# fakhirsh/path-tracer-python

Hardware: AMD Instinct MI355X
Metric: Msamples/s + achieved HBM GB/s, vol2_final_scene 800x800 at 1/2/4/8 MI355X (higher is better)
Workload: dtype f32; 1 GPU; vol2_final_scene 800x800 @ 16640 spp in total (260 steps x 64 spp), megakernel integrator, max_depth 50; scene=vol2_final_scene, width=800, height=800, variant=mk, traversal=stack, total_spp=16640, partition=tiles, rows_per_rank=800, max_depth=50, seed=0, parallelism=single GPU

## Files before the change

### path-tracer-python_amd/csrc/pt_abi.hip

```cpp
#include <hip/hip_runtime.h>

#include <cstdarg>
#include <cstdio>
#include <cstring>
#include <string>

#include "../../include/ptmi_wf_tiles.h"
#include "pt_args.hpp"
#include "pt_image.hpp"
#include "pt_launch.hpp"
#include "pt_prof.hpp"

namespace ptmi {

__global__ __launch_bounds__(kBlock) void clear_kernel(DevFrame fr, float* __restrict__ accum) {
  const int32_t npix = fr.w * fr.n_rows;
  for (int32_t i = (int32_t)(blockIdx.x * kBlock + threadIdx.x); i < npix; i += (int32_t)(gridDim.x * kBlock)) {
    int32_t lr = i / fr.w;
    int32_t px = fr.x0 + (i - lr * fr.w);
    int32_t py = frame_row(fr, lr);
    float* p = accum + 3 * ((size_t)py * (size_t)fr.width + (size_t)px);
    p[0] = 0.0f;
    p[1] = 0.0f;
    p[2] = 0.0f;
// ... 84 lines not shown
  if (s->shell != 0) {
    const int64_t off = ((int64_t)s->shell - 1) & ~(int64_t)1;
    if (s->shell < 0 || off % kNodeBytes != 0 || off / kNodeBytes >= s->n_inner)
      return fail(PTMI_EINVAL, "shell %d is not 1 + a node offset (multiple of %u, below %d nodes) + child index",
                  s->shell, kNodeBytes, s->n_inner);
  }
  std::memset(&d, 0, sizeof d);
  d.nodes = (const float4*)s->nodes;
  d.n_inner = s->n_inner;
  d.root_ref = (np > 0) ? s->root_ref : 0;
  for (int k = 0; k < 3; ++k) {
    d.root_min[k] = s->root_min[k];
    d.root_max[k] = s->root_max[k];
  }
  d.spheres = (const float4*)s->spheres;
  d.quads = (const float4*)s->quads;
  d.tris = (const float4*)s->tris;
  d.mats = (const float4*)s->mats;
  d.mat_base[kSphere] = 0;
  d.mat_base[kQuad] = s->num_spheres;
  d.mat_base[kTriangle] = s->num_spheres + s->num_quads;
  d.texels = s->texels;
  d.num_images = s->num_images;
  for (int k = 0; k < PTMI_MAX_IMAGES; ++k) {
    d.img_offset[k] = s->img_offset[k];
    d.img_w[k] = s->img_w[k];
    d.img_h[k] = s->img_h[k];
  }
  d.perlin_vec = (const float4*)s->perlin_vec;
  d.perlin_perm = s->perlin_perm;
  d.ref_nodes = (const float4*)s->ref_nodes;
  d.n_nodes = s->num_bvh_nodes;
  d.shell = s->max_leaf_depth <= 62 ? s->shell : 0;
  return PTMI_OK;
}

static int to_dev_frame(const ptmi_frame* f, DevFrame& d) {
  if (!f) return fail(PTMI_EINVAL, "frame is NULL");
  if (f->width <= 0 || f->height <= 0 || f->w <= 0 || f->h <= 0 || f->x0 < 0 || f->y0 < 0 ||
      f->x0 + f->w > f->width || f->y0 + f->h > f->height)
    return fail(PTMI_EINVAL, "bad window %d,%d %dx%d in %dx%d", f->x0, f->y0, f->w, f->h, f->width, f->height);
  if ((int64_t)f->width * (int64_t)f->height > (int64_t)0x7fffffff / 3)
    return fail(PTMI_ECAPACITY, "image too large");
  if (f->band_rows <= 0 || f->band_stride <= 0 || f->band_offset < 0 || f->band_offset >= f->band_stride)
    return fail(PTMI_EINVAL, "bad band partition");
  if (f->max_depth < 0 || f->max_depth > 255) return fail(PTMI_EINVAL, "max_depth must be in [0, 255]");
  std::memset(&d, 0, sizeof d);
  for (int k = 0; k < 3; ++k) {
    d.center[k] = f->cam.center[k];
    d.pixel00[k] = f->cam.pixel00[k];
    d.delta_u[k] = f->cam.delta_u[k];
    d.delta_v[k] = f->cam.delta_v[k];
    d.defocus_u[k] = f->cam.defocus_u[k];
    d.defocus_v[k] = f->cam.defocus_v[k];
    d.bg[k] = f->bg[k];
  }
  d.defocus_angle = f->cam.defocus_angle;
  d.max_depth = f->max_depth;
  d.seed = f->seed;
  d.width = f->width;
  d.height = f->height;
  d.x0 = f->x0;
  d.y0 = f->y0;
  d.w = f->w;
  d.h = f->h;
  d.band_rows = f->band_rows;
// ... 328 lines not shown
```

### path-tracer-python_amd/csrc/pt_device.hpp

```cpp
#pragma once
#include <hip/hip_runtime.h>
#include <stdint.h>

#include "../../include/ptmi.h"
#include "../../include/ptmi_math.h"
#include "../../include/ptmi_rng.h"

namespace ptmi {

constexpr float kTMin = 0.001f;
constexpr float kTMax = 1e10f;
constexpr int kRRMinDepth = 5;
constexpr float kRRMaxProb = 0.95f;
constexpr int kNumCounters = PTMI_NUM_COUNTERS;


struct FastDiv {
  uint64_t m;
  uint32_t sh, d;
};
static inline FastDiv fast_div(uint32_t d) {
  uint32_t l = 0;
  while ((1ull << l) < d) ++l;
  return FastDiv{((1ull << (32 + l)) / d) + 1ull, 32u + l, d};
}
__device__ __forceinline__ uint32_t fdiv(uint32_t n, const FastDiv& f) { return (uint32_t)(((uint64_t)n * f.m) >> f.sh); }
constexpr int kBlock = 256;

#ifndef PTMI_STRESS_WAVES
#define PTMI_STRESS_WAVES 0
#endif
constexpr int stress_waves(int w) { return PTMI_STRESS_WAVES > w ? PTMI_STRESS_WAVES : w; }

enum : int32_t { kSphere = 0, kTriangle = 1, kQuad = 2 };

struct DevScene {
  const float4* __restrict__ nodes;
  int32_t n_inner;
  int32_t root_ref;
  float root_min[3], root_max[3];
  const float4* __restrict__ spheres;
  const float4* __restrict__ quads;
  const float4* __restrict__ tris;
  const float4* __restrict__ mats;
  int32_t mat_base[3];
  const uint32_t* __restrict__ texels;
  int32_t num_images;
  int32_t img_offset[PTMI_MAX_IMAGES], img_w[PTMI_MAX_IMAGES], img_h[PTMI_MAX_IMAGES];
  const float4* __restrict__ perlin_vec;
  const int32_t* __restrict__ perlin_perm;
  const float4* __restrict__ ref_nodes;
  int32_t n_nodes;
  int32_t shell;
};

struct DevFrame {
  float center[3], pixel00[3], delta_u[3], delta_v[3], defocus_u[3], defocus_v[3];
  float defocus_angle;
  float bg[3];
  int32_t max_depth;
  uint32_t seed;
  int32_t width, height;
  int32_t x0, y0, w, h;
  int32_t band_rows, band_stride, band_offset;
  int32_t n_rows;
  int32_t traversal;
};

__device__ __forceinline__ int32_t leaf_type(int32_t ref) { return (ref >> 28) & 3; }
__device__ __forceinline__ int32_t leaf_index(int32_t ref) { return ref & 0x01ffffff; }
__device__ __forceinline__ int32_t leaf_class(int32_t ref) { return (ref >> 25) & 7; }

__device__ __forceinline__ int32_t frame_row(const DevFrame& fr, int32_t lr) {
  int32_t band = lr / fr.band_rows;
  int32_t within = lr - band * fr.band_rows;
  int32_t row = fr.y0 + (band * fr.band_stride + fr.band_offset) * fr.band_rows + within;
  return (row < fr.y0 + fr.h) ? row : -1;
}
// ... 86 lines not shown
  float z = sqrtf(1.0f - r2);
  float phi = PT_2PI_F * r1;
  float st = sqrtf(r2);
  float sp, cp;
  pt_sincosf(phi, &sp, &cp);
  float x = cp * st, y = sp * st;
  pt_v3 w = pt_normalize(n);
  pt_v3 a = (fabsf(w.x) < 0.9f) ? pt_v3f(1.0f, 0.0f, 0.0f)
            : (fabsf(w.y) < 0.9f) ? pt_v3f(0.0f, 1.0f, 0.0f) : pt_v3f(0.0f, 0.0f, 1.0f);
  pt_v3 v = pt_normalize(pt_cross(a, w));
  pt_v3 u = pt_cross(v, w);
  return pt_normalize(pt_add(pt_add(pt_scale(u, x), pt_scale(v, y)), pt_scale(w, z)));
}

__device__ __forceinline__ void get_ray(const DevFrame& fr, int32_t px, int32_t py, Rng& r, pt_v3& o,
                                        pt_v3& d) {
  float ox = r.next() - 0.5f;
  float oy = r.next() - 0.5f;
  pt_v3 p00 = pt_v3f(fr.pixel00[0], fr.pixel00[1], fr.pixel00[2]);
  pt_v3 du = pt_v3f(fr.delta_u[0], fr.delta_u[1], fr.delta_u[2]);
  pt_v3 dv = pt_v3f(fr.delta_v[0], fr.delta_v[1], fr.delta_v[2]);
  pt_v3 ps = pt_add(pt_add(p00, pt_scale(du, (float)px + ox)), pt_scale(dv, (float)py + oy));
  pt_v3 c = pt_v3f(fr.center[0], fr.center[1], fr.center[2]);
  o = c;
  if (fr.defocus_angle > 0.0f) {
    pt_v3 p = random_in_unit_disk(r);
    pt_v3 fu = pt_v3f(fr.defocus_u[0], fr.defocus_u[1], fr.defocus_u[2]);
    pt_v3 fv = pt_v3f(fr.defocus_v[0], fr.defocus_v[1], fr.defocus_v[2]);
    o = pt_add(pt_add(c, pt_scale(fu, p.x)), pt_scale(fv, p.y));
  }
  d = pt_sub(ps, o);
}

__device__ __forceinline__ bool pt_all4(bool a, bool b, bool c, bool d) {
  return __builtin_amdgcn_inverse_ballot_w64(__builtin_amdgcn_ballot_w64(a) & __builtin_amdgcn_ballot_w64(b) &
                                             __builtin_amdgcn_ballot_w64(c) & __builtin_amdgcn_ballot_w64(d));
}

__device__ __forceinline__ bool pt_all2(bool a, bool b) {
  return __builtin_amdgcn_inverse_ballot_w64(__builtin_amdgcn_ballot_w64(a) & __builtin_amdgcn_ballot_w64(b));
}


template <bool EXCL = false>
__device__ __forceinline__ bool hit_sphere_t(const float4 s, pt_v3 o, pt_v3 d, float tmin, float tmax,
                                             float& t) {
  pt_v3 c = pt_v3f(s.x, s.y, s.z);
  pt_v3 oc = pt_sub(c, o);
  float a = pt_dot(d, d);
  const float ra = pt_recip_for_div(a);
#define PT_SPH_DIV(x) pt_div_by((x), a, ra)
  float h = pt_dot(d, oc);
  float cc = pt_dot(oc, oc) - s.w * s.w;
  float disc = h * h - a * cc;
  if (disc >= 0.0f) {
    float sq = sqrtf(disc);
    float root = PT_SPH_DIV(h - sq);
    if (root < tmin || root > tmax) root = PT_SPH_DIV(h + sq);
    if (pt_all2(root >= tmin, EXCL ? root < tmax : root <= tmax)) { t = root; return true; }
  }
  return false;
#undef PT_SPH_DIV
}

template <bool EXCL = false>
__device__ __forceinline__ bool hit_quad_v(const float4 a, const float4 b, const float4 c, const float4 e, pt_v3 o,
                                           pt_v3 d, float tmin, float tmax, float& t) {
  pt_v3 n = pt_v3f(a.x, a.y, a.z);
  float denom = pt_dot(n, d);
  if (fabsf(denom) >= 1e-8f) {
    float tt = (a.w - pt_dot(n, o)) / denom;
    if (pt_all2(tt >= tmin, EXCL ? tt < tmax : tt <= tmax)) {
      pt_v3 Q = pt_v3f(b.x, b.y, b.z), u = pt_v3f(b.w, c.x, c.y), v = pt_v3f(c.z, c.w, e.x);
      pt_v3 w = pt_v3f(e.y, e.z, e.w);
      pt_v3 ip = pt_add(o, pt_scale(d, tt));
      pt_v3 pv = pt_sub(ip, Q);
      float alpha = pt_dot(w, pt_cross(pv, v));
      float beta = pt_dot(w, pt_cross(u, pv));
      if (pt_all4(alpha >= 0.0f, alpha <= 1.0f, beta >= 0.0f, beta <= 1.0f)) { t = tt; return true; }
    }
  }
  return false;
}

template <bool EXCL = false>
__device__ __forceinline__ bool hit_quad_t(const float4* __restrict__ q, pt_v3 o, pt_v3 d, float tmin,
                                           float tmax, float& t) {
  typedef float pt_f4 __attribute__((ext_vector_type(4)));
  pt_f4 A = ((const pt_f4*)q)[0], B = ((const pt_f4*)q)[1], C = ((const pt_f4*)q)[2], E = ((const pt_f4*)q)[3];
  asm volatile("" : "+v"(A), "+v"(B), "+v"(C), "+v"(E));
  return hit_quad_v<EXCL>(make_float4(A.x, A.y, A.z, A.w), make_float4(B.x, B.y, B.z, B.w),
                    make_float4(C.x, C.y, C.z, C.w), make_float4(E.x, E.y, E.z, E.w), o, d, tmin, tmax, t);
}

template <bool EXCL = false>
__device__ __forceinline__ bool hit_tri_v(const float4 a, const float4 b, const float4 c, pt_v3 o, pt_v3 d,
                                          float tmin, float tmax, float& t) {
  pt_v3 v0 = pt_v3f(a.x, a.y, a.z), e1 = pt_v3f(a.w, b.x, b.y), e2 = pt_v3f(b.z, b.w, c.x);
  pt_v3 hv = pt_cross(d, e2);
  float det = pt_dot(e1, hv);
  if (fabsf(det) >= 1e-8f) {
    float inv = 1.0f / det;
    pt_v3 s = pt_sub(o, v0);
    float u = inv * pt_dot(s, hv);
    if (pt_all2(u >= 0.0f, u <= 1.0f)) {
      pt_v3 q = pt_cross(s, e1);
      float v = inv * pt_dot(d, q);
      if (pt_all2(v >= 0.0f, u + v <= 1.0f)) {
        float tt = inv * pt_dot(e2, q);
        if (pt_all2(tt >= tmin, EXCL ? tt < tmax : tt <= tmax)) { t = tt; return true; }
      }
    }
  }
  return false;
}

template <bool EXCL = false>
__device__ __forceinline__ bool hit_tri_t(const float4* __restrict__ tr, pt_v3 o, pt_v3 d, float tmin,
                                          float tmax, float& t) {
  typedef float pt_f4 __attribute__((ext_vector_type(4)));
  pt_f4 A = ((const pt_f4*)tr)[0], B = ((const pt_f4*)tr)[1];
  pt_f4 C = ((const pt_f4*)tr)[2];
  asm volatile("" : "+v"(A), "+v"(B), "+v"(C));
  return hit_tri_v<EXCL>(make_float4(A.x, A.y, A.z, A.w), make_float4(B.x, B.y, B.z, B.w),
                         make_float4(C.x, C.y, C.z, C.w), o, d, tmin, tmax, t);
}

__device__ __forceinline__ bool hit_leaf(const DevScene& sc, int32_t ref, pt_v3 o, pt_v3 d, float tmin,
                                         float tmax, float& t) {
// ... 78 lines not shown
                                     float mxz, float tmin, float& E, float& X) {
  float t0x = (mnx - o.x) * inv.x, t1x = (mxx - o.x) * inv.x;
  float t0y = (mny - o.y) * inv.y, t1y = (mxy - o.y) * inv.y;
  float t0z = (mnz - o.z) * inv.z, t1z = (mxz - o.z) * inv.z;
  E = pt_maxf(pt_maxf(pt_minf(t0x, t1x), pt_minf(t0y, t1y)), pt_maxf(pt_minf(t0z, t1z), tmin));
  X = pt_minf(pt_minf(pt_maxf(t0x, t1x), pt_maxf(t0y, t1y)), pt_maxf(t0z, t1z));
}

__device__ __forceinline__ pt_f2 pt_f2s(float v) { return pt_f2{v, v}; }

#ifndef PTMI_PROBE
#define PTMI_PROBE 0
#endif
#if PTMI_PROBE
__device__ unsigned long long g_probe[16];
#endif

constexpr uint32_t kNodeBytes = 80;

struct Trav {
  pt_v3 inv;
  float tmin, closest;
  int32_t best;
  uint32_t sp;
  uint32_t sp0;
#if PTMI_PROBE == 2
  uint32_t probe;
#endif
  __device__ __forceinline__ bool any() const { return best != 0; }
  __device__ __forceinline__ bool busy() const { return sp != sp0; }
  __device__ __forceinline__ void init(Stack st) { sp = sp0 = lds_addr(st.slot0); }
};

template <int STACK, int SB = kBlock>
__device__ __forceinline__ void trav_begin(const DevScene& sc, Trav& tr, Stack st, pt_v3 d, pt_v3 o, float tmin,
                                           float tmax) {
  tr.inv = pt_v3f(fabsf(d.x) > 1e-8f ? 1.0f / d.x : 1e8f, fabsf(d.y) > 1e-8f ? 1.0f / d.y : 1e8f,
                  fabsf(d.z) > 1e-8f ? 1.0f / d.z : 1e8f);
  tr.tmin = tmin;
  tr.closest = tmax;
  tr.best = 0;
  tr.init(st);
  if (sc.n_inner == 0 && sc.root_ref >= 0) return;
  float E, X;
  slab(o, tr.inv, sc.root_min[0], sc.root_min[1], sc.root_min[2], sc.root_max[0], sc.root_max[1], sc.root_max[2],
       tmin, E, X);
  if (pt_minf(X, tr.closest) >= E) {
    lds_store2(tr.sp, (uint32_t)sc.root_ref, __float_as_uint(E));
    tr.sp += SB * 8;
  }
}

template <int STACK, int SB = kBlock, int DEFER = 0, int LDS = STACK>
__device__ __forceinline__ void trav_step(const DevScene& sc, const float4* node_base, Trav& tr, Stack st, pt_v3 o,
                                          pt_v3 d) {
  typedef float pt_f4 __attribute__((ext_vector_type(4)));
  typedef const __attribute__((address_space(1))) pt_f4 gf4;
  gf4* nodes = (gf4*)node_base;
  constexpr uint32_t kSlot = SB * 8;
  const uint32_t lim = tr.sp0 + (uint32_t)LDS * kSlot;
  tr.sp -= kSlot;
  const pt_u2v ent = stack_load<STACK, LDS, SB>(st, lim, tr.sp);
  const int32_t ref = (int32_t)ent.x;
  const unsigned long long m_leaf = pt_ballot(ref < 0), m_live = pt_ballot(__uint_as_float(ent.y) <= tr.closest);
  auto leaf_step = [&]() {
#if PTMI_PROBE == 2
    tr.probe |= leaf_type(ref) == kSphere ? 1 : 2;
#endif
    float t;
    const int32_t ty = leaf_type(ref), ix = leaf_index(ref);
    float tc = tr.closest;
    const unsigned long long m_s = pt_ballot(ty == kSphere), m_q = pt_ballot(ty == kQuad);
    if (__builtin_amdgcn_inverse_ballot_w64(m_s)) {
      if (hit_sphere_t<true>(sc.spheres[ix], o, d, tr.tmin, tr.closest, t)) tc = t;
    }
    if (__builtin_amdgcn_inverse_ballot_w64(m_q)) {
      if (hit_quad_t<true>(sc.quads + 4 * ix, o, d, tr.tmin, tr.closest, t)) tc = t;
    }
    if (__builtin_amdgcn_inverse_ballot_w64(~(m_s | m_q))) {
      if (hit_tri_t<true>(sc.tris + 3 * ix, o, d, tr.tmin, tr.closest, t)) tc = t;
    }
    if (tc < tr.closest) {
      tr.closest = tc;
// ... 606 lines not shown
```

### path-tracer-python_amd/csrc/pt_megakernel.hip

```cpp
#ifndef PTMI_PERLIN_UNROLL
#define PTMI_PERLIN_UNROLL 2
#endif
#include "pt_launch.hpp"
#include "pt_prof.hpp"

namespace ptmi {

enum : int32_t { kModeTrace = 0, kModeMediumExit = 1 };

struct PathState {
  pt_v3 o, dir, thr, color;
  Rng rng;
  int32_t depth;
  int32_t mode;
  float t_entry;
  int32_t ref_entry;
};

__device__ __forceinline__ void start_path(const DevFrame& fr, int32_t px, int32_t py, int32_t s,
                                           PathState& ps) {
  ps.rng.key = pt_path_key(fr.seed, (uint32_t)(py * fr.width + px), (uint32_t)s);
  ps.rng.n = 0;
  pt_v3 d;
  get_ray(fr, px, py, ps.rng, ps.o, d);
  ps.dir = pt_normalize(d);
  ps.thr = pt_v3f(1.0f, 1.0f, 1.0f);
  ps.color = pt_v3f(0.0f, 0.0f, 0.0f);
  ps.depth = 0;
  ps.mode = kModeTrace;
  ps.t_entry = 0.0f;
  ps.ref_entry = 0;
}

#ifndef PTMI_MK_SHADE_AT
#define PTMI_MK_SHADE_AT 24
#endif

#ifndef PTMI_MK_STEP_UNROLL
#define PTMI_MK_STEP_UNROLL 4
#endif

#ifndef PTMI_MK_PRIO_TRAV
#define PTMI_MK_PRIO_TRAV 2
#endif
#ifndef PTMI_MK_PRIO_SHADE
#define PTMI_MK_PRIO_SHADE 1
#endif
#ifndef PTMI_MK_PRIO_DRAIN
#define PTMI_MK_PRIO_DRAIN 0
#endif
#ifndef PTMI_MK_DEFER
#define PTMI_MK_DEFER 12
#endif
#ifndef PTMI_MK_MIN_WAVES
#define PTMI_MK_MIN_WAVES 4
#endif
#ifndef PTMI_MK_MIN_WAVES_16
#define PTMI_MK_MIN_WAVES_16 5
#endif

constexpr int kMkBlock = 64;

constexpr int kMkTile = 8;

template <int STACK, bool STAGED, int TRAV = PTMI_TRAV_STACK, bool LISTED = false, bool SHELL = false>
__global__ __launch_bounds__(kMkBlock, stress_waves(STACK < 20 ? PTMI_MK_MIN_WAVES_16 : STACK <= 20 ? PTMI_MK_MIN_WAVES : 1)) void mk_render_kernel(
    DevScene sc, DevFrame fr, float* __restrict__ accum, int32_t s_begin, int32_t s_count, int32_t chunk,
    float* __restrict__ staging, unsigned long long* __restrict__ counters, MkWork wk) {
  constexpr bool kPersist = STAGED;
  const float4* nodes = sc.nodes;
  {
    const uint64_t nb = (uint64_t)nodes;
    uint32_t lo = __builtin_amdgcn_readfirstlane((uint32_t)nb), hi = __builtin_amdgcn_readfirstlane((uint32_t)(nb >> 32));
    asm volatile("" : "+s"(lo), "+s"(hi));
    nodes = (const float4*)(((uint64_t)hi << 32) | lo);
  }
  __shared__ uint2 lds_stack[STACK * kMkBlock];
  const int tid = threadIdx.x;
  Stack st{lds_stack + tid};

  const int lane = tid & 63;
  const int32_t sq_x = fr.x0 + (int32_t)blockIdx.x * kMkTile;
  const int32_t sq_y = (int32_t)blockIdx.y * kMkTile;
  const size_t npix = (size_t)fr.w * (size_t)fr.n_rows;
  const pt_v3 bg = pt_v3f(fr.bg[0], fr.bg[1], fr.bg[2]);
  uint32_t n_seg = 0, n_med = 0, n_paths = 0;
  uint32_t n_rr = 0, n_cap = 0;
  PathState ps;

  const int32_t s0 = s_begin, ns = s_count;
  const uint32_t total = 64u * (uint32_t)ns;
  uint32_t next = 64u;
  uint32_t item = (uint32_t)lane;
  uint32_t wend = 0u;
  bool drained = false;
  int32_t px = 0, py = -1, lr = 0, s = s0;
// ... 19 lines not shown
                 s_begin + (int32_t)(j - tq * (uint32_t)wk.nb)};
    }
    return Loc{sq_x, sq_y, s0 + (int32_t)(k >> 6)};
  };
  auto bind = [&](uint32_t k) -> bool {
    const int32_t p = (int32_t)(k & 63u);
    const Loc l = locate(k);
    s = l.s;
    const int twl = kPersist ? wk.tw_log2 : 3;
    px = l.x + (p & ((1 << twl) - 1));
    lr = l.row + (p >> twl);
    py = (lr < fr.n_rows && px < fr.x0 + fr.w && s < s_begin + s_count) ? frame_row(fr, lr) : -1;
    if (STAGED) slot = (uint32_t)(s - s_begin) * (uint32_t)npix + (uint32_t)lr * (uint32_t)fr.w + (uint32_t)(px - fr.x0);
    return py >= 0;
  };
  if (kPersist) {
    next = 0u;
    item = 0xffffffffu;
  }
  if (!kPersist && item < total && bind(item)) {
    if (!STAGED) {
      ap = accum + 3 * ((size_t)py * (size_t)fr.width + (size_t)px);
      acc = pt_v3f(ap[0], ap[1], ap[2]);
    }
    start_path(fr, px, py, s, ps);
    live = true;
  }
  __syncthreads();

  typename TravOf<TRAV>::T tr;
  tr.init(st);
  bool trav = false;
  bool need_seg = false;
  auto begin_segment = [&]() {
    const bool em = ps.mode == kModeMediumExit;
    trav_begin<STACK, kMkBlock>(sc, tr, st, ps.dir, ps.o, em ? ps.t_entry + 0.0001f : kTMin, kTMax);
    if (em) ++n_med; else ++n_seg;
    trav = true;
  };
  if (live) begin_segment();

#if PTMI_PROBE == 4
  uint64_t p4[7] = {0, 0, 0, 0, 0, 0, 0};
  uint64_t p4_t = __builtin_amdgcn_s_memtime();
#define PT_P4(k)                                        \
  {                                                     \
    const uint64_t t_ = __builtin_amdgcn_s_memtime();   \
    p4[k] += t_ - p4_t;                                 \
    p4_t = t_;                                          \
  }
#else
#define PT_P4(k)
#endif
#if PTMI_PROBE == 3
  const uint64_t dr_t0 = __builtin_amdgcn_s_memtime();
  uint64_t dr_tdry = 0, dr_prev = 0, dr_lanecyc = 0;
  bool dr_dry = false;
#endif
#if PTMI_PROBE == 2
  uint64_t pr_trav = 0, pr_shade = 0, pr_steps = 0, pr_sph = 0, pr_oth = 0, pr_node = 0, pr_both = 0, pr_busy = 0;
  uint64_t pr_t = __builtin_amdgcn_s_memtime();
#endif
  for (;;) {
#if PTMI_MK_PRIO_TRAV >= 0
#if PTMI_MK_PRIO_DRAIN >= 0
    if (kPersist && drained && next >= wend)
      __builtin_amdgcn_s_setprio(PTMI_MK_PRIO_DRAIN);
    else
#endif
// ... 13 lines not shown
          trav_step<STACK, kMkBlock, PTMI_MK_DEFER>(sc, nodes, tr, st, ps.o, ps.dir);
#if PTMI_PROBE == 2
      ++pr_steps;
      pr_sph += pt_ballot(tr.probe & 1) ? 1 : 0;
      pr_oth += pt_ballot(tr.probe & 2) ? 1 : 0;
      pr_node += pt_ballot(tr.probe & 4) ? 1 : 0;
      pr_both += (pt_ballot(tr.probe & 1) && pt_ballot(tr.probe & 2)) ? 1 : 0;
      pr_busy += nbusy;
#endif
    }
#if PTMI_PROBE == 2
    {
      const uint64_t t = __builtin_amdgcn_s_memtime();
      pr_trav += t - pr_t;
      pr_t = t;
    }
#endif
#if PTMI_MK_PRIO_TRAV >= 0
    __builtin_amdgcn_s_setprio(PTMI_MK_PRIO_SHADE);
#endif
    PT_P4(0)
    const bool shade_now = trav && !tr.busy();
    const bool pn = shade_now && ps.mode != kModeMediumExit && tr.any() && leaf_class(tr.best) == PTMI_CLASS_NOISE;
    float pturb = 0.0f;
    if (pt_ballot(pn) != 0ull) pturb = perlin_turb3_wave(sc, pn, pt_add(ps.o, pt_scale(ps.dir, tr.closest)), lane);
    bool done = false, scattered = false, passthrough = false, to_medium = false;
    bool esc_miss = false;
    pt_v3 hp = pt_v3f(0.0f, 0.0f, 0.0f), sdir = hp, att = hp, n = hp;
    int32_t ruv = kRuvNone, sref = 0;
    float4 m0 = make_float4(0.0f, 0.0f, 0.0f, 0.0f);
    PT_P4(1)
    if (shade_now) {
      trav = false;
      bool exit_mode = ps.mode == kModeMediumExit;
      bool hit = tr.any();
      float t = tr.closest;
      const int32_t ref = tr.best;
      int32_t g = -1;
      Shell sh{};
      bool inl = false;
      if (!exit_mode) {
        if (!hit) {
          ps.color = pt_add(ps.color, pt_mul(ps.thr, bg));
          done = true;
        } else {
          g = mat_index(sc, ref);
          if (leaf_class(ref) == PTMI_CLASS_MEDIUM) {
            ps.t_entry = t;
            ps.ref_entry = ref;
            if constexpr (SHELL) {
              sh = load_shell_box(sc);
              if (ref == sh.ref && leaf_type(ref) == kSphere) {
                sh.sph = load_shell_sphere(sc, sh);
                const pt_v3 oc = pt_sub(ps.o, pt_v3f(sh.sph.x, sh.sph.y, sh.sph.z));
                inl = 4.0f * pt_dot(oc, oc) <= sh.sph.w * sh.sph.w;
              }
            }
            if (inl) {
              ++n_med;
              float te = kTMax;
              hit = shell_hit(sh, ps.o, ps.dir, tr.inv, t + 0.0001f, te);
              t = te;
              exit_mode = true;
            } else {
              ps.mode = kModeMediumExit;
              to_medium = true;
// ... 257 lines not shown
    }
    ap[0] = a0;
    ap[1] = a1;
    ap[2] = a2;
  }
}

hipError_t launch_stage_resolve(const DevFrame& fr, const float* staging, int32_t npix, int32_t batch,
                                float* accum, int prof_kind, hipStream_t stream) {
  unsigned g = (unsigned)((npix + kBlock - 1) / kBlock);
  if (g > 2048) g = 2048;
  const int pslot = prof_begin(prof_kind, stream);
  hipLaunchKernelGGL(stage_resolve, dim3(g), dim3(kBlock), 0, stream, fr, staging, npix, batch, accum);
  prof_end(pslot, stream);
  return hipGetLastError();
}

template <int STACK, int TRAV = PTMI_TRAV_STACK, bool SHELL = false>
static hipError_t launch_mk(const DevScene& sc, const DevFrame& fr, float* accum, int32_t s_begin,
                            int32_t s_count, unsigned long long* counters, hipStream_t stream) {
  dim3 grid((unsigned)((fr.w + kMkTile - 1) / kMkTile), (unsigned)((fr.n_rows + kMkTile - 1) / kMkTile));
  const int pslot = prof_begin(kProfMk, stream);
  hipLaunchKernelGGL((mk_render_kernel<STACK, false, TRAV, false, SHELL>), grid, dim3(kMkBlock), 0, stream, sc, fr, accum, s_begin,
                     s_count, s_count, (float*)nullptr, counters, MkWork{});
  prof_end(pslot, stream);
  return hipGetLastError();
}

template <int STACK, int TRAV>
constexpr bool kMkShellRung = TRAV == PTMI_TRAV_STACK && STACK >= 16 && STACK <= 20 && STACK != 19;

hipError_t mk_render(const DevScene& sc, const DevFrame& fr, int32_t stack_needed, float* accum,
                     int32_t s_begin, int32_t s_count, unsigned long long* counters, hipStream_t stream) {
  auto render = [&](auto shell) {
    return dispatch_traversal<false>(fr, stack_needed, [&](auto stack, auto trav) {
      constexpr int S = decltype(stack)::value, T = decltype(trav)::value;
      return launch_mk<S, T, decltype(shell)::value && kMkShellRung<S, T>>(sc, fr, accum, s_begin, s_count, counters,
                                                                         stream);
    });
  };
  if (sc.shell == 0) return render(std::false_type{});
  return render(std::true_type{});
}

template <int STACK, int TRAV = PTMI_TRAV_STACK, bool LISTED = false, bool SHELL = false>
static hipError_t launch_mk_trace(const DevScene& sc, const DevFrame& fr, float* staging, int32_t s_begin,
                                  int32_t nb, unsigned long long* counters, hipStream_t stream,
                                  const int32_t* tile_list, int32_t n_list) {
  float* accum = nullptr;
  int dev = 0, ncu = 0, per_cu = 0;
  hipError_t e0 = hipGetDevice(&dev);
  if (e0 == hipSuccess) e0 = hipDeviceGetAttribute(&ncu, hipDeviceAttributeMultiprocessorCount, dev);
  if (e0 == hipSuccess)
    e0 = hipOccupancyMaxActiveBlocksPerMultiprocessor(&per_cu, mk_render_kernel<STACK, true, TRAV, LISTED, SHELL>, kMkBlock, 0);
  if (e0 != hipSuccess) return e0;
  const MkPlan plan = mk_plan(fr, staging, nb, tile_list, n_list, per_cu, ncu);
  if (plan.err != hipSuccess) return plan.err;
  e0 = hipMemsetAsync(plan.wk.ctl, 0, plan.ctl_bytes, stream);
  if (e0 != hipSuccess) return e0;
  const int pslot = prof_begin(kProfMk, stream);
  hipLaunchKernelGGL((mk_render_kernel<STACK, true, TRAV, LISTED, SHELL>), dim3(plan.waves), dim3(kMkBlock), 0, stream,
                     sc, fr, accum, s_begin, nb, nb, staging, counters, plan.wk);
  prof_end(pslot, stream);
  return hipGetLastError();
}

hipError_t mk_trace_staged(const DevScene& sc, const DevFrame& fr, int32_t stack_needed, void* ws,
                           const int32_t* tile_list, int32_t n, int32_t s_begin, int32_t nb,
                           unsigned long long* counters, hipStream_t stream) {
  auto trace = [&](auto listed, auto shell) {
    return dispatch_traversal<true>(fr, stack_needed, [&](auto stack, auto trav) {
      constexpr int S = decltype(stack)::value, T = decltype(trav)::value;
      return launch_mk_trace<S, T, decltype(listed)::value, decltype(shell)::value && kMkShellRung<S, T>>(
          sc, fr, (float*)ws, s_begin, nb, counters, stream, tile_list, n);
    });
  };
  if (sc.shell == 0) {
    if (!tile_list) return trace(std::false_type{}, std::false_type{});
    return trace(std::true_type{}, std::false_type{});
  }
  if (!tile_list) return trace(std::false_type{}, std::true_type{});
  return trace(std::true_type{}, std::true_type{});
}

hipError_t mk_render_staged(const DevScene& sc, const DevFrame& fr, int32_t stack_needed, void* ws,
                            size_t ws_bytes, float* accum, int32_t s_begin, int32_t s_count,
                            unsigned long long* counters, hipStream_t stream) {
  if (s_count < 2)
    return mk_render(sc, fr, stack_needed, accum, s_begin, s_count, counters, stream);
  const int32_t npix = fr.w * fr.n_rows;
  const int32_t batch =
      fit_batch(s_count, mk_max_batch(fr), [&](int32_t b) { return mk_workspace_bytes(npix, b); }, ws_bytes);
  if (batch < 1) return hipErrorInvalidValue;
  for (int32_t b0 = 0; b0 < s_count; b0 += batch) {
    const int32_t nb = s_count - b0 < batch ? s_count - b0 : batch;
    hipError_t e = mk_trace_staged(sc, fr, stack_needed, ws, nullptr, 0, s_begin + b0, nb, counters, stream);
    if (e == hipSuccess) e = launch_stage_resolve(fr, (const float*)ws, npix, nb, accum, kProfMkResolve, stream);
    if (e != hipSuccess) return e;
  }
  return hipSuccess;
}

// ... 14 lines not shown
```

Baseline: 4214 Msamples/s.

## Pre-expand BVH chain to shell medium for rays starting inside it

Adds a shell-chain mechanism: for rays whose origin lies well inside the shell medium sphere, the traversal starts from the precomputed chain of BVH nodes leading to the shell leaf, pushing sibling subtrees directly instead of descending from the root. Where the chain is complete it skips pushing the shell subtree and tests the shell sphere analytically only if nothing else was hit. This is meant to remove the repeated root-to-shell descent. The stack request is raised for shell scenes, which may lower occupancy, and it adds a host checker tool.

```diff
diff --git a/path-tracer-python_amd/csrc/pt_abi.hip b/path-tracer-python_amd/csrc/pt_abi.hip
--- a/path-tracer-python_amd/csrc/pt_abi.hip
+++ b/path-tracer-python_amd/csrc/pt_abi.hip
@@ -140,6 +140,7 @@
   d.ref_nodes = (const float4*)s->ref_nodes;
   d.n_nodes = s->num_bvh_nodes;
   d.shell = s->max_leaf_depth <= 62 ? s->shell : 0;
+  d.max_leaf_depth = s->max_leaf_depth;
   return PTMI_OK;
 }
 
diff --git a/path-tracer-python_amd/csrc/pt_device.hpp b/path-tracer-python_amd/csrc/pt_device.hpp
--- a/path-tracer-python_amd/csrc/pt_device.hpp
+++ b/path-tracer-python_amd/csrc/pt_device.hpp
@@ -44,6 +44,7 @@
   const float4* __restrict__ tris;
   const float4* __restrict__ mats;
   int32_t mat_base[3];
+  int32_t max_leaf_depth;
   const uint32_t* __restrict__ texels;
   int32_t num_images;
   int32_t img_offset[PTMI_MAX_IMAGES], img_w[PTMI_MAX_IMAGES], img_h[PTMI_MAX_IMAGES];
@@ -196,18 +197,26 @@
   d = pt_sub(ps, o);
 }
 
-__device__ __forceinline__ bool pt_all4(bool a, bool b, bool c, bool d) {
+__host__ __device__ __forceinline__ bool pt_all4(bool a, bool b, bool c, bool d) {
+#if defined(__HIP_DEVICE_COMPILE__)
   return __builtin_amdgcn_inverse_ballot_w64(__builtin_amdgcn_ballot_w64(a) & __builtin_amdgcn_ballot_w64(b) &
                                              __builtin_amdgcn_ballot_w64(c) & __builtin_amdgcn_ballot_w64(d));
-}
-
-__device__ __forceinline__ bool pt_all2(bool a, bool b) {
+#else
+  return a && b && c && d;
+#endif
+}
+
+__host__ __device__ __forceinline__ bool pt_all2(bool a, bool b) {
+#if defined(__HIP_DEVICE_COMPILE__)
   return __builtin_amdgcn_inverse_ballot_w64(__builtin_amdgcn_ballot_w64(a) & __builtin_amdgcn_ballot_w64(b));
+#else
+  return a && b;
+#endif
 }
 
 
 template <bool EXCL = false>
-__device__ __forceinline__ bool hit_sphere_t(const float4 s, pt_v3 o, pt_v3 d, float tmin, float tmax,
+__host__ __device__ __forceinline__ bool hit_sphere_t(const float4 s, pt_v3 o, pt_v3 d, float tmin, float tmax,
                                              float& t) {
   pt_v3 c = pt_v3f(s.x, s.y, s.z);
   pt_v3 oc = pt_sub(c, o);
@@ -228,7 +237,7 @@
 }
 
 template <bool EXCL = false>
-__device__ __forceinline__ bool hit_quad_v(const float4 a, const float4 b, const float4 c, const float4 e, pt_v3 o,
+__host__ __device__ __forceinline__ bool hit_quad_v(const float4 a, const float4 b, const float4 c, const float4 e, pt_v3 o,
                                            pt_v3 d, float tmin, float tmax, float& t) {
   pt_v3 n = pt_v3f(a.x, a.y, a.z);
   float denom = pt_dot(n, d);
@@ -258,7 +267,7 @@
 }
 
 template <bool EXCL = false>
-__device__ __forceinline__ bool hit_tri_v(const float4 a, const float4 b, const float4 c, pt_v3 o, pt_v3 d,
+__host__ __device__ __forceinline__ bool hit_tri_v(const float4 a, const float4 b, const float4 c, pt_v3 o, pt_v3 d,
                                           float tmin, float tmax, float& t) {
   pt_v3 v0 = pt_v3f(a.x, a.y, a.z), e1 = pt_v3f(a.w, b.x, b.y), e2 = pt_v3f(b.z, b.w, c.x);
   pt_v3 hv = pt_cross(d, e2);
@@ -403,23 +412,32 @@
   __device__ __forceinline__ void init(Stack st) { sp = sp0 = lds_addr(st.slot0); }
 };
 
-template <int STACK, int SB = kBlock>
-__device__ __forceinline__ void trav_begin(const DevScene& sc, Trav& tr, Stack st, pt_v3 d, pt_v3 o, float tmin,
-                                           float tmax) {
+__device__ __forceinline__ void trav_ray(Trav& tr, Stack st, pt_v3 d, float tmin, float tmax) {
   tr.inv = pt_v3f(fabsf(d.x) > 1e-8f ? 1.0f / d.x : 1e8f, fabsf(d.y) > 1e-8f ? 1.0f / d.y : 1e8f,
                   fabsf(d.z) > 1e-8f ? 1.0f / d.z : 1e8f);
   tr.tmin = tmin;
   tr.closest = tmax;
   tr.best = 0;
   tr.init(st);
+}
+
+template <int STACK, int SB = kBlock>
+__device__ __forceinline__ void trav_root(const DevScene& sc, Trav& tr, pt_v3 o) {
   if (sc.n_inner == 0 && sc.root_ref >= 0) return;
   float E, X;
   slab(o, tr.inv, sc.root_min[0], sc.root_min[1], sc.root_min[2], sc.root_max[0], sc.root_max[1], sc.root_max[2],
-       tmin, E, X);
+       tr.tmin, E, X);
   if (pt_minf(X, tr.closest) >= E) {
     lds_store2(tr.sp, (uint32_t)sc.root_ref, __float_as_uint(E));
     tr.sp += SB * 8;
   }
+}
+
+template <int STACK, int SB = kBlock>
+__device__ __forceinline__ void trav_begin(const DevScene& sc, Trav& tr, Stack st, pt_v3 d, pt_v3 o, float tmin,
+                                           float tmax) {
+  trav_ray(tr, st, d, tmin, tmax);
+  trav_root<STACK, SB>(sc, tr, o);
 }
 
 template <int STACK, int SB = kBlock, int DEFER = 0, int LDS = STACK>
diff --git a/path-tracer-python_amd/csrc/pt_megakernel.hip b/path-tracer-python_amd/csrc/pt_megakernel.hip
--- a/path-tracer-python_amd/csrc/pt_megakernel.hip
+++ b/path-tracer-python_amd/csrc/pt_megakernel.hip
@@ -3,6 +3,7 @@
 #endif
 #include "pt_launch.hpp"
 #include "pt_prof.hpp"
+#include "pt_shell_chain.hpp"
 
 namespace ptmi {
 
@@ -62,6 +63,13 @@
 constexpr int kMkBlock = 64;
 
 constexpr int kMkTile = 8;
+
+struct ChainLoad {
+  const float4* nodes;
+  __device__ __forceinline__ uint32_t operator()(uint32_t off, uint32_t i) const {
+    return *(const __attribute__((address_space(4))) uint32_t*)((uintptr_t)nodes + off + 4u * i);
+  }
+};
 
 template <int STACK, bool STAGED, int TRAV = PTMI_TRAV_STACK, bool LISTED = false, bool SHELL = false>
 __global__ __launch_bounds__(kMkBlock, stress_waves(STACK < 20 ? PTMI_MK_MIN_WAVES_16 : STACK <= 20 ? PTMI_MK_MIN_WAVES : 1)) void mk_render_kernel(
@@ -147,9 +155,40 @@
   tr.init(st);
   bool trav = false;
   bool need_seg = false;
+  ShellChain chain{};
+  ShellPlan cplan{0, false};
+  float4 csph = make_float4(0.0f, 0.0f, 0.0f, 0.0f);
+  const ChainLoad cld{sc.nodes};
+  if constexpr (SHELL) {
+    chain = shell_chain_find(cld, sc.shell, sc.n_inner, sc.root_ref);
+    cplan = shell_chain_plan(chain, STACK, sc.max_leaf_depth);
+    if (cplan.m > 0) {
+      const Shell sh = load_shell_box(sc);
+      if (sh.ref < 0 && leaf_type(sh.ref) == kSphere && leaf_class(sh.ref) == PTMI_CLASS_MEDIUM)
+        csph = load_shell_sphere(sc, sh);
+      else
+        cplan = ShellPlan{0, false};
+    }
+  }
   auto begin_segment = [&]() {
     const bool em = ps.mode == kModeMediumExit;
-    trav_begin<STACK, kMkBlock>(sc, tr, st, ps.dir, ps.o, em ? ps.t_entry + 0.0001f : kTMin, kTMax);
+    const float tmin = em ? ps.t_entry + 0.0001f : kTMin;
+    bool root = true;
+    if constexpr (SHELL) {
+      if (cplan.m > 0) {
+        root = false;
+        trav_ray(tr, st, ps.dir, tmin, kTMax);
+        const pt_v3 oc = pt_sub(ps.o, pt_v3f(csph.x, csph.y, csph.z));
+        bool ex = false;
+        if (4.0f * pt_dot(oc, oc) <= csph.w * csph.w)
+          ex = shell_chain_begin(cld, chain, cplan, ps.o, ps.dir, tr.inv, tr.tmin, tr.closest, [&](uint32_t ref, float E) {
+            lds_store2(tr.sp, ref, __float_as_uint(E));
+            tr.sp += kMkBlock * 8;
+          });
+        if (!ex) trav_root<STACK, kMkBlock>(sc, tr, ps.o);
+      }
+    }
+    if (root) trav_begin<STACK, kMkBlock>(sc, tr, st, ps.dir, ps.o, tmin, kTMax);
     if (em) ++n_med; else ++n_seg;
     trav = true;
   };
@@ -229,6 +268,20 @@
     PT_P4(1)
     if (shade_now) {
       trav = false;
+      if constexpr (SHELL) {
+        if (cplan.skip && !tr.any()) {
+          const pt_v3 oc = pt_sub(ps.o, pt_v3f(csph.x, csph.y, csph.z));
+          if (4.0f * pt_dot(oc, oc) <= csph.w * csph.w) {
+            Shell s0 = load_shell_box(sc);
+            s0.sph = csph;
+            float te;
+            if (shell_hit(s0, ps.o, ps.dir, tr.inv, tr.tmin, te)) {
+              tr.closest = te;
+              tr.best = s0.ref;
+            }
+          }
+        }
+      }
       bool exit_mode = ps.mode == kModeMediumExit;
       bool hit = tr.any();
       float t = tr.closest;
@@ -552,6 +605,7 @@
 
 hipError_t mk_render(const DevScene& sc, const DevFrame& fr, int32_t stack_needed, float* accum,
                      int32_t s_begin, int32_t s_count, unsigned long long* counters, hipStream_t stream) {
+  if (sc.shell != 0) stack_needed = shell_chain_stack_request(stack_needed);
   auto render = [&](auto shell) {
     return dispatch_traversal<false>(fr, stack_needed, [&](auto stack, auto trav) {
       constexpr int S = decltype(stack)::value, T = decltype(trav)::value;
@@ -588,6 +642,7 @@
 hipError_t mk_trace_staged(const DevScene& sc, const DevFrame& fr, int32_t stack_needed, void* ws,
                            const int32_t* tile_list, int32_t n, int32_t s_begin, int32_t nb,
                            unsigned long long* counters, hipStream_t stream) {
+  if (sc.shell != 0) stack_needed = shell_chain_stack_request(stack_needed);
   auto trace = [&](auto listed, auto shell) {
     return dispatch_traversal<true>(fr, stack_needed, [&](auto stack, auto trav) {
       constexpr int S = decltype(stack)::value, T = decltype(trav)::value;
diff --git a/path-tracer-python_amd/csrc/pt_shell_chain.hpp b/path-tracer-python_amd/csrc/pt_shell_chain.hpp
--- /dev/null
+++ b/path-tracer-python_amd/csrc/pt_shell_chain.hpp
@@ -0,0 +1,165 @@
+#pragma once
+#include <stdint.h>
+
+#include "../../include/ptmi_math.h"
+
+namespace ptmi {
+
+constexpr int kShellChainMax = 6;
+constexpr uint32_t kChainNodeBytes = 80;
+
+struct ShellChain {
+  uint32_t off[kShellChainMax];
+  uint32_t side;
+  int32_t m;
+  bool full;
+};
+
+PT_HD float pt_chain_f(uint32_t b) {
+  union {
+    uint32_t u;
+    float f;
+  } v;
+  v.u = b;
+  return v.f;
+}
+PT_HD uint32_t pt_chain_u(float f) {
+  union {
+    uint32_t u;
+    float f;
+  } v;
+  v.f = f;
+  return v.u;
+}
+
+template <class L>
+PT_HD ShellChain shell_chain_find(const L& ld, int32_t shell, int32_t n_inner, int32_t root_ref) {
+  ShellChain ch{};
+  if (shell <= 0 || n_inner <= 0 || root_ref < 0) return ch;
+  const uint32_t v = (uint32_t)shell - 1u, pc = v & 1u, poff = v & ~1u;
+  const uint32_t end = (uint32_t)n_inner * kChainNodeBytes;
+  if (poff >= end) return ch;
+  uint32_t box[7];
+#pragma unroll
+  for (int a = 0; a < 7; ++a) box[a] = ld(poff, 2u * (uint32_t)a + pc + (a == 6 ? 2u : 0u));
+  uint32_t cur = (uint32_t)root_ref;
+  bool go = true;
+#pragma unroll
+  for (int k = 0; k < kShellChainMax; ++k) {
+    if (go) {
+      go = false;
+      if (cur < end) {
+        bool m0 = true, m1 = true;
+#pragma unroll
+        for (int a = 0; a < 7; ++a) {
+          const uint32_t i = 2u * (uint32_t)a + (a == 6 ? 2u : 0u);
+          m0 = m0 && ld(cur, i) == box[a];
+          m1 = m1 && ld(cur, i + 1u) == box[a];
+        }
+        if (m0 != m1) {
+          const uint32_t c = m1 ? 1u : 0u;
+          const int32_t ref = (int32_t)ld(cur, 12u + c);
+          if (cur == poff) {
+            if (c == pc) {
+              ch.off[k] = cur;
+              ch.side |= c << k;
+              ch.m = k + 1;
+              ch.full = true;
+            }
+          } else if (ref >= 0) {
+            ch.off[k] = cur;
+            ch.side |= c << k;
+            ch.m = k + 1;
+            cur = (uint32_t)ref;
+            go = true;
+          }
+        }
+      }
+    }
+  }
+  return ch;
+}
+
+PT_HD int32_t shell_chain_slots(int32_t max_leaf_depth, int32_t m, bool skip) {
+  return max_leaf_depth + m - (skip ? 1 : 0);
+}
+
+struct ShellPlan {
+  int32_t m;
+  bool skip;
+};
+
+PT_HD ShellPlan shell_chain_plan(const ShellChain& ch, int32_t stack, int32_t max_leaf_depth) {
+  ShellPlan p{0, false};
+  if (ch.m < 1) return p;
+  if (ch.full && shell_chain_slots(max_leaf_depth, ch.m, true) <= stack) {
+    p.m = ch.m;
+    p.skip = true;
+    return p;
+  }
+  const int32_t fit = stack - max_leaf_depth;
+  p.m = ch.m < fit ? ch.m : fit;
+  if (p.m < 1) p.m = 0;
+  return p;
+}
+
+#ifndef PTMI_SHELL_CHAIN_EXTRA
+#define PTMI_SHELL_CHAIN_EXTRA (kShellChainMax - 2)
+#endif
+PT_HD int32_t shell_chain_stack_request(int32_t stack_needed) {
+  if (stack_needed > 20) return stack_needed;
+  int32_t want = stack_needed + PTMI_SHELL_CHAIN_EXTRA;
+  if (want >= 19) want = 20;
+  return want;
+}
+
+template <class L, class P>
+PT_HD bool shell_chain_begin(const L& ld, const ShellChain& ch, const ShellPlan& p, pt_v3 o, pt_v3 d, pt_v3 inv,
+                             float tmin, float tmax, P&& push) {
+  auto slab1 = [&](uint32_t off, uint32_t c, float& E, float& X, float& dist) {
+    const float lox = pt_chain_f(ld(off, 0u + c)), loy = pt_chain_f(ld(off, 2u + c)), loz = pt_chain_f(ld(off, 4u + c));
+    const float hix = pt_chain_f(ld(off, 6u + c)), hiy = pt_chain_f(ld(off, 8u + c)), hiz = pt_chain_f(ld(off, 10u + c));
+    const float cz = pt_chain_f(ld(off, 14u + c));
+    const float t0x = (lox - o.x) * inv.x, t1x = (hix - o.x) * inv.x;
+    const float t0y = (loy - o.y) * inv.y, t1y = (hiy - o.y) * inv.y;
+    const float t0z = (loz - o.z) * inv.z, t1z = (hiz - o.z) * inv.z;
+    E = pt_maxf(pt_maxf(pt_minf(t0x, t1x), pt_minf(t0y, t1y)), pt_maxf(pt_minf(t0z, t1z), tmin));
+    X = pt_minf(pt_minf(pt_maxf(t0x, t1x), pt_maxf(t0y, t1y)), pt_maxf(t0z, t1z));
+    const float cx = (lox + hix) * 0.5f, cy = (loy + hiy) * 0.5f;
+    dist = ((cx - o.x) * d.x + (cy - o.y) * d.y) + (cz - o.z) * d.z;
+  };
+  float Eg, Xg, dg;
+  slab1(ch.off[0], ch.side & 1u, Eg, Xg, dg);
+  if (!(pt_minf(Xg, tmax) >= Eg)) return false;
+  uint32_t ref[kShellChainMax];
+  float E[kShellChainMax];
+  bool far_[kShellChainMax], near_[kShellChainMax];
+  uint32_t rest = 0u;
+#pragma unroll
+  for (int k = 0; k < kShellChainMax; ++k) {
+    far_[k] = near_[k] = false;
+    ref[k] = 0u;
+    E[k] = 0.0f;
+    if (k < p.m) {
+      const uint32_t c = (ch.side >> k) & 1u, s = c ^ 1u;
+      float X, ds;
+      slab1(ch.off[k], s, E[k], X, ds);
+      ref[k] = ld(ch.off[k], 12u + s);
+      const bool hit = X >= E[k];
+      const bool nr = s == 0u ? ds < dg : !(dg < ds);
+      near_[k] = hit && nr;
+      far_[k] = hit && !nr;
+      if (k == p.m - 1) rest = ld(ch.off[k], 12u + c);
+    }
+  }
+#pragma unroll
+  for (int k = 0; k < kShellChainMax; ++k)
+    if (far_[k]) push(ref[k], E[k]);
+  if (!p.skip) push(rest, Eg);
+#pragma unroll
+  for (int k = kShellChainMax - 1; k >= 0; --k)
+    if (near_[k]) push(ref[k], E[k]);
+  return true;
+}
+
+}
diff --git a/path-tracer-python_amd/csrc/shell_chain_check.cpp b/path-tracer-python_amd/csrc/shell_chain_check.cpp
--- /dev/null
+++ b/path-tracer-python_amd/csrc/shell_chain_check.cpp
@@ -0,0 +1,230 @@
+#include <stdint.h>
+#include <stdio.h>
+#include <stdlib.h>
+
+#include <vector>
+
+#include "pt_check_io.hpp"
+#include "pt_device.hpp"
+#include "pt_shell_chain.hpp"
+
+using namespace ptmi;
+
+namespace {
+
+constexpr int kCap = 256;
+
+struct Scene {
+  std::vector<float> nodes, spheres, quads, tris;
+  int32_t shell, n_inner, root_ref, max_leaf_depth;
+};
+
+struct Load {
+  const std::vector<float>* nodes;
+  uint32_t operator()(uint32_t off, uint32_t i) const { return pt_chain_u((*nodes)[off / 4u + i]); }
+};
+
+struct Entry {
+  uint32_t ref;
+  float E;
+};
+
+struct Walk {
+  pt_v3 o, d, inv;
+  float tmin, closest;
+  int32_t best;
+  std::vector<Entry> st;
+  int peak;
+  bool overflow;
+  void push(uint32_t ref, float E) {
+    if ((int)st.size() >= kCap) {
+      overflow = true;
+      return;
+    }
+    st.push_back(Entry{ref, E});
+    if ((int)st.size() > peak) peak = (int)st.size();
+  }
+};
+
+float4 f4(const std::vector<float>& v, size_t i) { return make_float4(v[i], v[i + 1], v[i + 2], v[i + 3]); }
+
+void ray(Walk& w, pt_v3 o, pt_v3 d, float tmin) {
+  w.o = o;
+  w.d = d;
+  w.inv = pt_v3f(fabsf(d.x) > 1e-8f ? 1.0f / d.x : 1e8f, fabsf(d.y) > 1e-8f ? 1.0f / d.y : 1e8f,
+                 fabsf(d.z) > 1e-8f ? 1.0f / d.z : 1e8f);
+  w.tmin = tmin;
+  w.closest = kTMax;
+  w.best = 0;
+  w.st.clear();
+  w.peak = 0;
+  w.overflow = false;
+}
+
+void slab6(const Walk& w, const float* b, int c, float& E, float& X) {
+  const float t0x = (b[0 + c] - w.o.x) * w.inv.x, t1x = (b[6 + c] - w.o.x) * w.inv.x;
+  const float t0y = (b[2 + c] - w.o.y) * w.inv.y, t1y = (b[8 + c] - w.o.y) * w.inv.y;
+  const float t0z = (b[4 + c] - w.o.z) * w.inv.z, t1z = (b[10 + c] - w.o.z) * w.inv.z;
+  E = pt_maxf(pt_maxf(pt_minf(t0x, t1x), pt_minf(t0y, t1y)), pt_maxf(pt_minf(t0z, t1z), w.tmin));
+  X = pt_minf(pt_minf(pt_maxf(t0x, t1x), pt_maxf(t0y, t1y)), pt_maxf(t0z, t1z));
+}
+
+void run(const Scene& sc, Walk& w) {
+  while (!w.st.empty()) {
+    const Entry e = w.st.back();
+    w.st.pop_back();
+    if (!(e.E <= w.closest)) continue;
+    const int32_t ref = (int32_t)e.ref;
+    if (ref < 0) {
+      const int32_t ty = (ref >> 28) & 3, ix = ref & 0x01ffffff;
+      float t, tc = w.closest;
+      if (ty == kSphere) {
+        if (hit_sphere_t<true>(f4(sc.spheres, 4 * (size_t)ix), w.o, w.d, w.tmin, w.closest, t)) tc = t;
+      } else if (ty == kQuad) {
+        const size_t q = 16 * (size_t)ix;
+        if (hit_quad_v<true>(f4(sc.quads, q), f4(sc.quads, q + 4), f4(sc.quads, q + 8), f4(sc.quads, q + 12), w.o, w.d,
+                             w.tmin, w.closest, t))
+          tc = t;
+      } else {
+        const size_t q = 12 * (size_t)ix;
+        if (hit_tri_v<true>(f4(sc.tris, q), f4(sc.tris, q + 4), f4(sc.tris, q + 8), w.o, w.d, w.tmin, w.closest, t)) tc = t;
+      }
+      if (tc < w.closest) {
+        w.closest = tc;
+        w.best = ref;
+      }
+      continue;
+    }
+    const float* b = &sc.nodes[(size_t)ref / 4];
+    float E0, X0, E1, X1;
+    slab6(w, b, 0, E0, X0);
+    slab6(w, b, 1, E1, X1);
+    const float cx0 = (b[0] + b[6]) * 0.5f, cx1 = (b[1] + b[7]) * 0.5f;
+    const float cy0 = (b[2] + b[8]) * 0.5f, cy1 = (b[3] + b[9]) * 0.5f;
+    const float d0 = ((cx0 - w.o.x) * w.d.x + (cy0 - w.o.y) * w.d.y) + (b[14] - w.o.z) * w.d.z;
+    const float d1 = ((cx1 - w.o.x) * w.d.x + (cy1 - w.o.y) * w.d.y) + (b[15] - w.o.z) * w.d.z;
+    const bool ln = d0 < d1, h0 = X0 >= E0, h1 = X1 >= E1;
+    const uint32_t r0 = pt_chain_u(b[12]), r1 = pt_chain_u(b[13]);
+    if (ln) {
+      if (h1) w.push(r1, E1);
+      if (h0) w.push(r0, E0);
+    } else {
+      if (h0) w.push(r0, E0);
+      if (h1) w.push(r1, E1);
+    }
+  }
+}
+
+void begin_root(const Scene& sc, Walk& w) {
+  if (sc.n_inner == 0 && sc.root_ref >= 0) return;
+  if (sc.root_ref < 0) {
+    w.push((uint32_t)sc.root_ref, w.tmin);
+    return;
+  }
+  const float* b = &sc.nodes[(size_t)sc.root_ref / 4];
+  float u[12];
+  for (int a = 0; a < 3; ++a) {
+    u[2 * a] = pt_minf(b[2 * a], b[2 * a + 1]);
+    u[6 + 2 * a] = pt_maxf(b[6 + 2 * a], b[6 + 2 * a + 1]);
+  }
+  float E, X;
+  slab6(w, u, 0, E, X);
+  if (pt_minf(X, w.closest) >= E) w.push((uint32_t)sc.root_ref, E);
+}
+
+}
+
+int main(int argc, char** argv) {
+  if (argc != 12) {
+    fprintf(stderr, "usage: %s SHELL N_INNER ROOT_REF MAX_LEAF_DEPTH STACK nodes spheres quads tris rays out\n", argv[0]);
+    return 2;
+  }
+  Scene sc;
+  sc.shell = atoi(argv[1]);
+  sc.n_inner = atoi(argv[2]);
+  sc.root_ref = atoi(argv[3]);
+  sc.max_leaf_depth = atoi(argv[4]);
+  const int32_t stack = atoi(argv[5]);
+  std::vector<float> rays;
+  if (!read_all_f32(argv[6], sc.nodes) || !read_all_f32(argv[7], sc.spheres) || !read_all_f32(argv[8], sc.quads) ||
+      !read_all_f32(argv[9], sc.tris) || !read_all_f32(argv[10], rays)) {
+    fprintf(stderr, "cannot read the inputs\n");
+    return 2;
+  }
+  if (sc.n_inner < 0 || sc.nodes.size() < (size_t)sc.n_inner * (kChainNodeBytes / 4) || rays.size() % 7 != 0 ||
+      sc.spheres.size() % 4 != 0 || sc.quads.size() % 16 != 0 || sc.tris.size() % 12 != 0) {
+    fprintf(stderr, "input sizes do not fit\n");
+    return 2;
+  }
+  const Load ld{&sc.nodes};
+  const ShellChain ch = shell_chain_find(ld, sc.shell, sc.n_inner, sc.root_ref);
+  const ShellPlan pl = shell_chain_plan(ch, stack, sc.max_leaf_depth);
+  printf("chain m %d full %d side %u plan m %d skip %d slots %d off", ch.m, ch.full ? 1 : 0, ch.side, pl.m,
+         pl.skip ? 1 : 0, pl.m ? shell_chain_slots(sc.max_leaf_depth, pl.m, pl.skip) : sc.max_leaf_depth + 1);
+  for (int k = 0; k < ch.m; ++k) printf(" %u", ch.off[k]);
+  printf("\n");
+
+  float4 sph = make_float4(0.0f, 0.0f, 0.0f, 0.0f);
+  const float* pbox = nullptr;
+  int pc = 0;
+  if (pl.m > 0) {
+    const uint32_t v = (uint32_t)sc.shell - 1u;
+    pc = (int)(v & 1u);
+    pbox = &sc.nodes[(v & ~1u) / 4];
+    const int32_t ref = (int32_t)pt_chain_u(pbox[12 + pc]);
+    const size_t ix = (size_t)(ref & 0x01ffffff);
+    if (ref >= 0 || ((ref >> 28) & 3) != kSphere || 4 * ix + 4 > sc.spheres.size()) {
+      fprintf(stderr, "the hint does not point at a sphere leaf\n");
+      return 2;
+    }
+    sph = f4(sc.spheres, 4 * ix);
+  }
+
+  const size_t n = rays.size() / 7;
+  std::vector<uint32_t> out(8 * n);
+  bool overflow = false;
+  Walk w;
+  for (size_t r = 0; r < n; ++r) {
+    const float* q = &rays[7 * r];
+    const pt_v3 o = pt_v3f(q[0], q[1], q[2]), d = pt_v3f(q[3], q[4], q[5]);
+    uint32_t* res = &out[8 * r];
+    ray(w, o, d, q[6]);
+    begin_root(sc, w);
+    run(sc, w);
+    overflow = overflow || w.overflow;
+    res[0] = (uint32_t)w.best, res[1] = pt_chain_u(w.closest), res[2] = (uint32_t)w.peak;
+    ray(w, o, d, q[6]);
+    bool gate = false, expanded = false, finished = false;
+    if (pl.m > 0) {
+      const pt_v3 oc = pt_sub(o, pt_v3f(sph.x, sph.y, sph.z));
+      gate = 4.0f * pt_dot(oc, oc) <= sph.w * sph.w;
+    }
+    if (gate)
+      expanded = shell_chain_begin(ld, ch, pl, w.o, w.d, w.inv, w.tmin, w.closest,
+                                   [&](uint32_t ref, float E) { w.push(ref, E); });
+    if (!expanded) begin_root(sc, w);
+    run(sc, w);
+    if (pl.skip && gate && w.best == 0) {
+      finished = true;
+      float E, X, t;
+      slab6(w, pbox, pc, E, X);
+      if (pt_minf(X, kTMax) >= E && hit_sphere_t<true>(sph, w.o, w.d, w.tmin, kTMax, t)) {
+        w.closest = t;
+        w.best = (int32_t)pt_chain_u(pbox[12 + pc]);
+      }
+    }
+    overflow = overflow || w.overflow;
+    res[3] = (uint32_t)w.best, res[4] = pt_chain_u(w.closest), res[5] = (uint32_t)w.peak;
+    res[6] = expanded ? 1u : 0u, res[7] = finished ? 1u : 0u;
+  }
+  FILE* f = fopen(argv[11], "wb");
+  if (!f || fwrite(out.data(), sizeof(uint32_t), out.size(), f) != out.size() || fclose(f) != 0) {
+    fprintf(stderr, "cannot write %s\n", argv[11]);
+    return 2;
+  }
+  if (overflow) {
+    fprintf(stderr, "a walk needed more than %d slots\n", kCap);
+    return 1;
+  }
+  return 0;
+}
```

Measured after the change: 4343 Msamples/s, median of 6. +3.1%, better.
